# andrewcsmith/vox_box.rs

Hardware: AMD Instinct MI355X
Metric: frames/sec (pitch+LPC+formants), 48 kHz 25 ms/10 ms hop, 1→8 MI355X (higher is better)
Workload: dtype f64

## Files before the change

vox_box.rs_amd/csrc/vbx_pitch_refine.hpp:

```cpp
#pragma once
#include <type_traits>

#include "vbx_device.hpp"
#include "vbx_kernels.hpp"

namespace vbx {


__device__ __forceinline__ double fma_sc(double p, double x, const double c) {
    double r;
    asm("v_fma_f64 %0, %1, %2, %3" : "=v"(r) : "v"(p), "v"(x), "s"(c));
    return r;
}

__device__ __forceinline__ double sin_poly_q(double x) {
    const double x2 = x * x;
    double p = -1.9572941063391261231e-20;
    p = fma_sc(p, x2, 8.2206352466243297170e-18);
    p = fma_sc(p, x2, -2.8114572543455207632e-15);
    p = fma_sc(p, x2, 7.6471637318198164759e-13);
    p = fma_sc(p, x2, -1.6059043836821614599e-10);
    p = fma_sc(p, x2, 2.5052108385441718775e-08);
    p = fma_sc(p, x2, -2.7557319223985890653e-06);
    p = fma_sc(p, x2, 1.9841269841269841270e-04);
// ... 450 lines not shown
            if (rest & 3) sinc_stream_tail<NSTEP>(s, step, rest & 3);
        } else if (sel) run_set(s, c1);
        else run_set(s, c0);
        const double acc = s.acc0 + s.acc1;
        const double signed_acc = __hiloint2double(__double2hiint(acc) ^ sign_bit, __double2loint(acc));
        return group_sum<64>(signed_acc * k);
    };
    double v = readfirstlane_f64(a + golden * (b - a));
    double fv = eval(v);
    double x = v, w = v, fx = fv, fw = fv;
    const bool prunable = __any(a >= (double)(-offset));
    pruned = false;
    if (prunable && __any(((fv <= 1.) ? fv : 1.) < bar)) { pruned = true; terms += nterms_s; evals += nevals_s; return true; }
    for (int it = 1; it <= 60; it++) {
        const double range = b - a;
        const double middle_range = (a + b) * 0.5;
        const double tol_act = sqrt_epsilon * fabs(x) + tol / 3.;
        if (__any(fabs(x - middle_range) + range * 0.5 <= 2. * tol_act)) break;
        double new_step = __any(x < middle_range) ? golden * (b - x) : golden * (a - x);
        if (__any(fabs(x - w) >= tol_act)) {
            const double t = (x - w) * (fx - fv);
            double q = (x - v) * (fx - fw);
            double p = (x - v) * q - (x - w) * t;
            q = 2. * q - t;
            if (__any(q > 0.)) p = -p; else q = -q;
            if (__any((int)(fabs(p) < fabs(new_step * q)) & (int)(p > q * (a - x + 2. * tol_act)) & (int)(p < q * (b - x - 2. * tol_act)))) {
                asm volatile("" ::: "memory");
                new_step = p / q;
            }
        }
        if (__any(fabs(new_step) < tol_act)) new_step = __any(new_step > 0.) ? tol_act : -tol_act;
        const double t = readfirstlane_f64(x + new_step);
        const double ft = eval(t);
        nevals_s += 1u;
        if (__any(ft <= fx)) {
            if (__any(t < x)) { asm volatile(""); b = x; } else { asm volatile(""); a = x; }
            v = w; w = x; x = t;
            fv = fw; fw = fx; fx = ft;
        } else {
            if (__any(t < x)) { asm volatile(""); a = t; } else { asm volatile(""); b = t; }
            if (__any(ft <= fw || fabs(w - x) < eps)) {
                v = w; w = t;
                fv = fw; fw = ft;
            } else if (__any(ft <= fv || fabs(v - x) < eps || fabs(v - w) < eps)) {
                v = t;
                fv = ft;
            }
        }
        if (prunable && __any(fx < bar)) { pruned = true; break; }
    }
    terms += nterms_s; evals += nevals_s;
    if (!pruned) { xmid = x; ymid = fx; }
    return true;
}

constexpr int Y_PAD = 16;
#ifndef VBX_EXP_PB
#define VBX_EXP_PB 5
#endif
constexpr int PB = VBX_EXP_PB;
__device__ __forceinline__ double block_abs_sum(const double *yp) {
    double s = fabs(yp[0]) + fabs(yp[1]);
#pragma unroll
    for (int i = 2; i + 1 < PB; i += 2) s += fabs(yp[i]) + fabs(yp[i + 1]);
    if (PB & 1) s += fabs(yp[PB - 1]);
    return s;
}
typedef unsigned short cand_t;
constexpr int PG = 16;
constexpr int PNG = 64 / PG;
constexpr int GROUP_PATH_MIN_CAND = 32;
#ifndef VBX_EXP_RG
#define VBX_EXP_RG 16
#endif
#ifndef VBX_EXP_GROUP_KMAX
#define VBX_EXP_GROUP_KMAX 4
#endif
constexpr int RG = VBX_EXP_RG;
#ifndef VBX_EXP_DUAL_MIN_CAND
#define VBX_EXP_DUAL_MIN_CAND 6
#endif
constexpr int DUAL_MIN_CAND = VBX_EXP_DUAL_MIN_CAND;

__device__ __forceinline__ void cand_from_peak(const double *ys, int kk, double sample_rate, int offset,
                                               double &freq, double &nn, const bool f32 = false) {
    const double peak = ys[kk], peak_rev = ys[kk - 1], peak_fwd = ys[kk + 1];
    if (f32) {
#pragma clang fp contract(off)
        const double dr = 0.5 * (double)(float)(peak_fwd - peak_rev);
        const double d2r = 2. * peak - (double)(float)(peak_rev - peak_fwd);
        freq = (double)(float)(sample_rate / (double)(float)((double)kk + dr / d2r));
        nn = (double)(float)((double)(float)(sample_rate / freq) - (double)offset);
        return;
    }
    const double dr = 0.5 * (peak_fwd - peak_rev);
    const double d2r = 2. * peak - (peak_rev - peak_fwd);
    freq = sample_rate / ((double)kk + dr / d2r);
    nn = sample_rate / freq - (double)offset;
}

constexpr int BOUND_HEAD = 8;

__device__ __forceinline__ double taper_upper(double theta) {
    const double t = theta * theta;
    double p = fma(t, 2.48015873015873016e-05, -1.38888888888888894e-03);
    p = fma(p, t, 4.16666666666666644e-02);
    p = fma(p, t, -0.5);
    return fma(0.5, fma(p, t, 1.0), 0.5) * (1.0 + 1.0e-15);
}

__device__ __forceinline__ void abs_range_idx(int nblk, int i0, int i1, int &j0, int &j1) {
    i0 = (i0 < 0) ? 0 : i0;
    const int last = PB * nblk - 1;
    i1 = (i1 > last) ? last : i1;
    const bool empty = i1 < i0;
    j0 = empty ? 0 : (int)((unsigned)i0 / PB);
    j1 = empty ? 0 : (int)((unsigned)i1 / PB) + 1;
}
template <int STEP, int TB>
__device__ __forceinline__ double first_eval_tail(const double *p16, int nblk, int offset, int nl, int nr, int D, int lo0,
                                                  double phil, double phir, double hl, double hr) {
    double tail = 0.0;
    for (int lo = lo0; lo <= D;) {
        double sl[TB], sr[TB];
#pragma unroll
        for (int q = 0, l = lo; q < TB; q++, l *= STEP) {
            const int hi = (2 * l < D + 1) ? 2 * l : D + 1;
            int a0 = 0, a1 = 0, b0 = 0, b1 = 0;
            if (l <= D) {
                abs_range_idx(nblk, offset + nr - (hi - 1), offset + nr - l, a0, a1);
                abs_range_idx(nblk, offset + nl + l, offset + nl + hi - 1, b0, b1);
            }
            sl[q] = p16[a1] - p16[a0];
            sr[q] = p16[b1] - p16[b0];
        }
#pragma unroll
        for (int q = 0; q < TB; q++) {
            if (lo > D) break;
            const double pl = phil + (double)lo, pr = phir + (double)lo;
            const double cl = rcp_nr1(pl) * taper_upper(hl * pl);
            const double cr = rcp_nr1(pr) * taper_upper(hr * pr);
            tail = fma(cl, sl[q], tail);
            tail = fma(cr, sr[q], tail);
            lo *= STEP;
        }
    }
    return tail;
}

__device__ __forceinline__ double first_eval_bound(const double *ys, const double *p16, int nblk, int nvalid, int ylen,
                                                   int offset, int nx, double nn, int depth) {
    const double INF = __builtin_inf();
    if (nn == 0. || nn >= (double)nx || !(nn - 1. < nn + 1.)) return INF;
    double v0;
    {
#pragma clang fp contract(off)
        const double golden = 1. - 0.6180339887498948482045868343656381177203091798057628621;
        const double ba = nn - 1., bb = nn + 1.;
        if (!(ba >= (double)(-offset))) return INF;
        v0 = ba + golden * (bb - ba);
    }
    if (nx < 1 || v0 > (double)nx || v0 < 0.0) return INF;
    const double fl = floor(v0);
    const int nl = (int)fl, nr = nl + 1;
    const double phil = v0 - (double)nl, phir = 1.0 - phil;
    if (fabs(v0 - (double)nl) < 1.0e-10 || fabs(v0 - (double)nr) < 1.0e-10) return INF;
    int D = depth;
    if ((offset + nr) < D) D = ((offset + nr) < 0) ? 0 : (offset + nr);
    if ((offset + nl + D) >= nx) D = nx - offset + nl - 1;
    if (D < 0 || offset + nr >= ylen || D > offset + nr || offset + nl < 0 || offset + nl + D >= ylen) return INF;
    const double s0 = sin_poly(M_PI * fmin(phil, phir)) * 0.31830988618379067154;
    const double hl = M_PI * rcp_nr1(phil + (double)D), hr = M_PI * rcp_nr1(phir + (double)D);
    double head = 0.0;
    const int nh = (BOUND_HEAD < D + 1) ? BOUND_HEAD : D + 1;
    {
        double cl = cos_0_pi(hl * phil), cr = cos_0_pi(hr * phir);
        double dl = cos_0_pi(hl * (phil + 1.0)) - cl, dr = cos_0_pi(hr * (phir + 1.0)) - cr;
        const double sl = sin_poly(0.5 * hl), sr = sin_poly(0.5 * hr);
        const double kl = 4.0 * sl * sl, kr = 4.0 * sr * sr;
        double yl[BOUND_HEAD], yr[BOUND_HEAD];
#pragma unroll
// ... 15 lines not shown
        }
    }
    head *= s0;
    double tail = first_eval_tail<2, 4>(p16, nblk, offset, nl, nr, D, nh, phil, phir, hl, hr);
    tail *= s0;
    const double ub = head + tail * (1.0 + 1.0e-9) + (1.0e-9 + 1.0e-11 * p16[nblk]);
    return (ub != ub) ? INF : ub;
}

__device__ __forceinline__ double first_eval_bound_quad(const double *ys, const double *p16, int nblk, int nvalid, int ylen,
                                                        int offset, int nx, double nn, int depth, int sub, bool have) {
    const double INF = __builtin_inf();
    bool inf = !have;
    double v0 = 0.;
    if (!inf) {
        if (nn == 0. || nn >= (double)nx || !(nn - 1. < nn + 1.)) inf = true;
        else {
#pragma clang fp contract(off)
            const double golden = 1. - 0.6180339887498948482045868343656381177203091798057628621;
            const double ba = nn - 1., bb = nn + 1.;
            if (!(ba >= (double)(-offset))) inf = true;
            v0 = ba + golden * (bb - ba);
        }
    }
    if (!inf && (nx < 1 || v0 > (double)nx || v0 < 0.0)) inf = true;
    int nl = 0, nr = 1, D = 0;
    double phil = 0.5, phir = 0.5;
    if (!inf) {
        const double fl = floor(v0);
        nl = (int)fl; nr = nl + 1;
        phil = v0 - (double)nl; phir = 1.0 - phil;
        if (fabs(v0 - (double)nl) < 1.0e-10 || fabs(v0 - (double)nr) < 1.0e-10) inf = true;
        D = depth;
        if ((offset + nr) < D) D = ((offset + nr) < 0) ? 0 : (offset + nr);
        if ((offset + nl + D) >= nx) D = nx - offset + nl - 1;
        if (D < 0 || offset + nr >= ylen || D > offset + nr || offset + nl < 0 || offset + nl + D >= ylen) inf = true;
    }
    double head = 0.0, tail = 0.0;
    if (!inf) {
        const double s0 = sin_poly(M_PI * fmin(phil, phir)) * 0.31830988618379067154;
        const double hl = M_PI * rcp_nr1(phil + (double)D), hr = M_PI * rcp_nr1(phir + (double)D);
        const int nh = (BOUND_HEAD < D + 1) ? BOUND_HEAD : D + 1;
        double yl[BOUND_HEAD / 4], yr[BOUND_HEAD / 4];
#pragma unroll
        for (int j = 0; j < BOUND_HEAD / 4; j++) {
            const int m = sub + 4 * j;
            const bool in = m < nh;
            yl[j] = y_at_padded(ys, nvalid, in ? offset + nr - m : 0);
            yr[j] = y_at_padded(ys, nvalid, in ? offset + nl + m : 0);
        }
#pragma unroll
        for (int j = 0; j < BOUND_HEAD / 4; j++) {
            const int m = sub + 4 * j;
            if (m >= nh) break;
            const double pl = phil + (double)m, pr = phir + (double)m;
            const double tl = yl[j] * rcp_nr1(pl) * fma(0.5, cos_0_pi(hl * pl), 0.5);
            const double tr = yr[j] * rcp_nr1(pr) * fma(0.5, cos_0_pi(hr * pr), 0.5);
            const double t = tl + tr;
            head += (m & 1) ? -t : t;
        }
        head *= s0;
        tail = first_eval_tail<16, 2>(p16, nblk, offset, nl, nr, D, nh << sub, phil, phir, hl, hr);
        tail *= s0;
    }
    head = group_sum<4>(head);
    tail = group_sum<4>(tail);
    const double ub = head + tail * (1.0 + 1.0e-9) + (1.0e-9 + 1.0e-11 * p16[nblk]);
    return (inf || ub != ub) ? INF : ub;
}

__device__ __forceinline__ int pick_best(float *keys, int ncand, double bar, int lane) {
    double bv = -__builtin_inf(); int bi = 0x7fffffff;
    for (int i = lane; i < ncand; i += 64) { const double v = (double)keys[i]; if (v > bv) { bv = v; bi = i; } }
    const double gm = wave_max(bv);
    int pick = (bv == gm) ? bi : 0x7fffffff;
    for (int o = 32; o > 0; o >>= 1) { const int other = __shfl_xor(pick, o, 64); pick = (other < pick) ? other : pick; }
    if (pick == 0x7fffffff || !(gm >= bar)) return -1;
    if (lane == 0) keys[pick] = -__builtin_inff();
    wave_sync();
    return pick;
}


__device__ __forceinline__ int pick_best_pred(float *keys, const cand_t *cand_list, const double *ys, int ncand, double bar, int lane) {
    double bv = -__builtin_inf(); int bi = 0x7fffffff;
    for (int i = lane; i < ncand; i += 64) {
        const float kv = keys[i];
        if (kv > -__builtin_inff() && (double)kv >= bar) {
            const int k = (int)cand_list[i];
            double p = fmin(ys[k - 1], ys[k + 1]);
            if (!(p == p)) p = __builtin_inf();
            if (bi == 0x7fffffff || p > bv) { bv = p; bi = i; }
        }
    }
    const double gm = wave_max(bv);
    int pick = (bi != 0x7fffffff && bv == gm) ? bi : 0x7fffffff;
    for (int o = 32; o > 0; o >>= 1) { const int other = __shfl_xor(pick, o, 64); pick = (other < pick) ? other : pick; }
    if (pick == 0x7fffffff) return -1;
    if (lane == 0) keys[pick] = -__builtin_inff();
    wave_sync();
    return pick;
}


__host__ __device__ constexpr int pitch_refine_lds_bytes(int n, int nst = 0, int cap = 0) {
    const int m = (nst > 0) ? nst : n;
    return (m + Y_PAD + ((((m + PB - 1) / PB) + 2) & ~1)) * 8 + ((cap > 0) ? cap : n / 4 + 8) * (int)(sizeof(float) + sizeof(cand_t));
}

inline int pitch_curve_reach(int n, double sample_rate, double fmin) {
    if (!(fmin > 0.0) || !(sample_rate > 0.0)) return 0;
    const double reach = 2.0 * ceil(sample_rate / fmin) + 16.0;
    if (!(reach < (double)n)) return 0;
    return ((int)reach + 1) & ~1;
}
inline int pitch_curve_entries(int n, double sample_rate, double fmin) {
    if ((n & 1) || !(fmin > 0.0) || !(sample_rate > 0.0)) return 0;
    const double reach = 2.0 * ceil(sample_rate / fmin) + 16.0;
    if (!(reach < (double)n)) return 0;
    int m = (int)reach;
    if (m < n / 2 + 2) m = n / 2 + 2;
    m = (m + 1) & ~1;
    return (m < n) ? m : 0;
}

struct pitch_params_t { double sample_rate, threshold, fmin, fmax; int kmax; int full_off; int f32 = 0; int ncurve = 0; };
__host__ __device__ constexpr int pitch_full_list_entries(int n) { return n / 4 + 2; }

#ifndef VBX_EXP_CELL_NB_PITCH
#define VBX_EXP_CELL_NB_PITCH 0
#endif
#ifndef VBX_EXP_CELL_NB_REFINE_LIST
#define VBX_EXP_CELL_NB_REFINE_LIST 3
#endif
constexpr int PITCH_CELL_NB = VBX_EXP_CELL_NB_PITCH, REFINE_LIST_CELL_NB = VBX_EXP_CELL_NB_REFINE_LIST;
template <int STAGE = 0, int NB = 0>
__device__ __forceinline__ bool pitch_refine_store(double *ys, int n, const pitch_params_t &pp, long f,
                                                   double *__restrict__ out_cand, long cand_ld,
                                                   int32_t *__restrict__ out_count, int32_t *__restrict__ status,
                                                   unsigned long long *__restrict__ work, double unc_tol = 0.0,
                                                   double2 *full = nullptr, int *io_ncand = nullptr, int cand_cap = 0,
                                                   uint16_t *list_at = nullptr) {
    const int lane = lane_id();
    const double sample_rate = pp.sample_rate, threshold = pp.threshold, fmin = pp.fmin, fmax = pp.fmax;
    const int kmax = pp.kmax;
    const bool f32 = pp.f32 != 0;
    const int nst = (pp.ncurve > 0) ? pp.ncurve : n;
    const int nblk = (nst + PB - 1) / PB;
    double *p16 = ys + nst + Y_PAD;
    float *keys = reinterpret_cast<float *>(p16 + ((nblk + 2) & ~1));
    cand_t *cand_list = (STAGE == 1 && list_at != nullptr) ? reinterpret_cast<cand_t *>(list_at)
                                                           : reinterpret_cast<cand_t *>(keys + ((STAGE == 2 && cand_cap > 0) ? cand_cap : n / 4 + 8));
    const int b = (int)floor(0.5 * (double)n);
    const int offset = -b - 1;
    const int nx = b - offset;
    const int ylen = 2 * n;
    const int nvalid = nst + Y_PAD;

    VBX_PHASE_INIT();
    int ncand = 0;
    if constexpr (STAGE == 2) ncand = *io_ncand;
    else {
    int npeak = 0;
    bool unsure = false;
    for (int base = 0; base < b; base += 64) {
        const int k = base + lane;
        bool peak = false;
        if (k >= 1 && k + 1 < b) {
            const double c = ys[k];
            const double d1 = c - ys[k - 1], d2 = c - ys[k + 1];
            peak = (ys[k - 1] < c) && (ys[k + 1] < c);
            unsure = unsure || (fabs((d1 < d2) ? d1 : d2) <= unc_tol);
        }
        const unsigned long long mask = __ballot(peak);
        if (peak) cand_list[npeak + __popcll(mask & ((1ull << lane) - 1ull))] = (cand_t)k;
        npeak += __popcll(mask);
    }
    wave_sync();
    if (unc_tol > 0.0 && __any(unsure)) return false;
    VBX_PHASE(work, f, 6);
    unsure = false;
    for (int base = 0; base < npeak; base += 64) {
        const int i = base + lane;
        bool pass = false;
        int k = 0;
        if (i < npeak) {
            k = cand_list[i];
            double freq, nn;
            cand_from_peak(ys, k, sample_rate, offset, freq, nn, f32);
            pass = (freq == 0.0) || (freq > fmin && freq < fmax);
            if (unc_tol > 0.0) {
                const double c = ys[k], d2r = 2. * c - (ys[k - 1] - ys[k + 1]), dr = 0.5 * (ys[k + 1] - ys[k - 1]);
                const double dlag = unc_tol * (1.0 + 4.0 * fabs(dr / d2r)) / fabs(d2r);
                const double tol_f = 2.0 * freq * dlag / fabs((double)k + dr / d2r);
                if (!(fabs(freq - fmin) > tol_f && fabs(freq - fmax) > tol_f)) unsure = true;
            }
        }
        wave_sync();
        const unsigned long long mask = __ballot(pass);
        if (pass) cand_list[ncand + __popcll(mask & ((1ull << lane) - 1ull))] = (cand_t)k;
        ncand += __popcll(mask);
        wave_sync();
    }

    if (unc_tol > 0.0 && __any(unsure)) return false;
    VBX_PHASE(work, f, 7);
    }
    if constexpr (STAGE == 1) { *io_ncand = ncand; return true; }

    const bool in_order = full != nullptr || kmax > ncand || f32;
    if (!in_order) {
        const int per = (nblk + 63) >> 6;
        double tot = 0.0;
        for (int q = 0; q < per; q++) {
            const int j = lane * per + q;
            if (j < nblk) tot += block_abs_sum(ys + PB * j);
        }
        const double incl = wave_inclusive_scan(tot);
        double run = incl - tot;
        if (lane == 0) p16[0] = 0.0;
        for (int q = 0; q < per; q++) {
            const int j = lane * per + q;
            if (j < nblk) {
                run += block_abs_sum(ys + PB * j);
                p16[j + 1] = run;
            }
        }
        wave_sync();
        const bool quad = ((ncand + 15) / 16) * 7 < ((ncand + 63) / 64) * 25;
        if (quad) {
            for (int base = 0; base < ncand; base += 16) {
                const int c = base + (lane >> 2);
                const bool have = c < ncand;
                double freq = 0., nn = 0.;
                if (have) cand_from_peak(ys, cand_list[c], sample_rate, offset, freq, nn, f32);
                const double ub = first_eval_bound_quad(ys, p16, nblk, nvalid, ylen, offset, nx, nn, 1200, lane & 3, have);
                const double kb = (ub <= 1.) ? ub : ((ub != ub) ? __builtin_inf() : ((ub == __builtin_inf()) ? ub : 1.));
                if (have && (lane & 3) == 0) keys[c] = __double2float_ru(kb);
            }
        } else {
            for (int c = lane; c < ncand; c += 64) {
                double freq, nn;
                cand_from_peak(ys, cand_list[c], sample_rate, offset, freq, nn, f32);
                const double ub = first_eval_bound(ys, p16, nblk, nvalid, ylen, offset, nx, nn, 1200);
                const double kb = (ub <= 1.) ? ub : ((ub != ub) ? __builtin_inf() : ((ub == __builtin_inf()) ? ub : 1.));
                keys[c] = __double2float_ru(kb);
            }
        }
        wave_sync();
    }

    VBX_PHASE(work, f, 8);
    int st = 0;
    int kept = 0;
    double lf = 0.0, ls = 0.0;
    bool any_nan = false;
    int li = 0;
    { lf = 0.0; ls = threshold; li = ncand; kept = 1; }
    const bool fullm = full != nullptr;
    if (fullm && lane == 0) full[ncand] = double2{0.0, threshold};

#define VBX_BAR() ((!fullm && !f32 && kept == kmax) ? readlane_f64(ls, kmax - 1) : -__builtin_inf())
    auto insert = [&](double f_g, double s_g, int c_g) {
        if (s_g != s_g) any_nan = true;
        if (fullm) { if (lane == 0) full[c_g] = double2{f_g, s_g}; return; }
        const int pos = __popcll(__ballot(lane < kept && (ls > s_g || (ls == s_g && li < c_g))));
        const double pf = from_prev_lane(lf), ps = from_prev_lane(ls);
        const int pi = __builtin_amdgcn_update_dpp(0, li, DPP_WAVE_SHR1, 0xf, 0xf, true);
        if (lane > pos) { lf = pf; ls = ps; li = pi; }
        if (lane == pos) { lf = f_g; ls = s_g; li = c_g; }
        kept = (kept + 1 < kmax) ? kept + 1 : kmax;
    };
    unsigned cterms = 0, cevals = 0;

    int next_full = ncand - 1;
    unsigned nterms = 0, nevals = 0;
    int group_lanes = RG;
    if (ncand <= GROUP_PATH_MIN_CAND && !(kmax >= VBX_EXP_GROUP_KMAX && ncand >= 4)) {
        auto enter = [&](int c, double xmid, double ymid) __attribute__((always_inline)) {
            double xm, ym;
            {
#pragma clang fp contract(off)
                xm = xmid + (double)offset;
                ym = ymid;
                if (ym > 1.) ym = 1. / ym;
                xm = sample_rate / (f32 ? (double)(float)xm : xm);
                if (f32) { xm = (double)(float)xm; ym = (double)(float)ym; }
            }
            insert(xm, ym, c);
        };
        int c_general = -1;
#ifndef VBX_EXP_NO_WAVE_BRENT
        for (;;) {
            const double bar = VBX_BAR();
            const int c = in_order ? next_full-- : pick_best_pred(keys, cand_list, ys, ncand, bar, lane);
            if (c < 0) break;
            double freq, nn, xmid, ymid;
            cand_from_peak(ys, cand_list[c], sample_rate, offset, freq, nn, f32);
            bool dropped = false;
            if (__builtin_expect(!improve_extremum_sinc_wave<NB>(ys, nvalid, ylen, offset, nx, nn, 1200, xmid, ymid, cterms, cevals, bar, dropped), 0)) {
                c_general = c;
                break;
            }
            if (dropped) continue;
            enter(c, xmid, ymid);
        }
        if (c_general >= 0)
#endif
        for (;;) {
            const double bar = VBX_BAR();
            int c = c_general;
            c_general = -1;
            if (c < 0) c = in_order ? next_full-- : pick_best_pred(keys, cand_list, ys, ncand, bar, lane);
            if (c < 0) break;
            double freq, nn, xmid, ymid;
            cand_from_peak(ys, cand_list[c], sample_rate, offset, freq, nn, f32);
            bool dropped = false;
            improve_extremum_sinc<64>(ys, nvalid, ylen, offset, nx, nn, 1200, true, xmid, ymid, st, &cterms, &cevals, bar, &dropped);
            if (dropped) continue;
            enter(c, xmid, ymid);
        }
    } else {
      auto run_groups = [&](auto pg_tag, auto dual_tag) {
        constexpr int PG = decltype(pg_tag)::value;
        constexpr bool DUAL = decltype(dual_tag)::value;
        bool exhausted = false;
        const int gid = lane / PG;
        int ci = -1, it = 0;
        bool special = false, safe = false, trusted = false;
        double ba = 0., bb = 0., v = 0., w = 0., x = 0., fv = 0., fw = 0., fx = 0., xmid = 0., ymid = 0.;
        constexpr unsigned long long LEADERS = (PG == 16) ? 0x0001000100010001ull : (PG == 8) ? 0x0101010101010101ull
                                             : (PG == 32) ? 0x0000000100000001ull : (PG == 4) ? 0x1111111111111111ull : 1ull;
        const double golden = 1. - 0.6180339887498948482045868343656381177203091798057628621;
        const double sqrt_epsilon = 1.4901161193847656e-08, eps = 2.220446049250313e-16, tol = 1e-10;
        for (;;) {
#pragma clang fp contract(off)
            bool finished = false;
            double range = 0., middle_range = 0., tol_act = 0.;
            if (ci >= 0) {
                if (special) finished = true;
                else if (it > 0) {
                    range = bb - ba;
                    middle_range = (ba + bb) * 0.5;
                    tol_act = sqrt_epsilon * fabs(x) + tol / 3.;
                    if (it > 60 || fabs(x - middle_range) + range * 0.5 <= 2. * tol_act) { finished = true; xmid = x; ymid = fx; }
                }
            }
            if (__any(finished)) {
                unsigned long long fm = __ballot(finished) & LEADERS;
                double xm = xmid + (double)offset;
                double ym = ymid;
                if (ym > 1.) ym = 1. / ym;
                double cf = sample_rate / (f32 ? (double)(float)xm : xm), cs = ym;
                if (f32) { cf = (double)(float)cf; cs = (double)(float)cs; }
                while (fm) {
                    const int ld = __builtin_ctzll(fm);
                    fm &= fm - 1;
                    insert(readlane_f64(cf, ld), readlane_f64(cs, ld), __builtin_amdgcn_readlane(ci, ld));
                }
                if (finished) ci = -1;
            }
            {
                unsigned long long im = __ballot(ci < 0) & LEADERS;
                while (im != 0ull && !exhausted) {
                    const int c = in_order ? next_full-- : pick_best_pred(keys, cand_list, ys, ncand, VBX_BAR(), lane);
                    if (c < 0) { exhausted = true; break; }
                    const int g = __builtin_ctzll(im) / PG;
                    im &= im - 1ull;
                    if (gid == g) {
                        ci = c;
                        double freq, nn;
                        cand_from_peak(ys, cand_list[ci], sample_rate, offset, freq, nn, f32);
                        it = 0; special = false; xmid = 0.; ymid = 0.;
                        if (nn == 0.) { special = true; xmid = 0.; ymid = ys[0]; }
                        else if (nn >= (double)nx) { special = true; xmid = (double)nx; ymid = y_at(ys, nvalid, nx - 1); }
                        else if (!(nn - 1. < nn + 1.)) { special = true; st |= 4; }
                        ba = nn - 1.; bb = nn + 1.;
                        safe = ba >= (double)(-offset);
                        trusted = !special && sinc_bracket_trusted(ba, bb, nvalid, ylen, offset, nx, 1200);
                    }
                }
            }
            if (!__any(ci >= 0)) break;
            const double bar = VBX_BAR();

            bool need = false;
            double t = 0.;
            if (ci >= 0 && !special) {
                if (it == 0) { v = ba + golden * (bb - ba); t = v; }
                else {
                    double new_step = (x < middle_range) ? golden * (bb - x) : golden * (ba - x);
                    if (fabs(x - w) >= tol_act) {
                        const double tt = (x - w) * (fx - fv);
                        double q = (x - v) * (fx - fw);
                        double pp = (x - v) * q - (x - w) * tt;
                        q = 2. * q - tt;
                        if (q > 0.) pp = -pp; else q = -q;
                        if (fabs(pp) < fabs(new_step * q) && pp > q * (ba - x + 2. * tol_act) && pp < q * (bb - x - 2. * tol_act))
                            new_step = pp / q;
                    }
                    if (fabs(new_step) < tol_act) new_step = (new_step > 0.) ? tol_act : -tol_act;
                    t = x + new_step;
                }
                need = true;
            }
            const double ft = sinc_interp<PG, DUAL>(ys, nvalid, ylen, offset, nx, t, 1200, need, st, &nterms, trusted);
            nevals += need ? 1u : 0u;
            if (need) {
                if (it == 0) {
                    x = v; w = v; fv = ft; fx = ft; fw = ft; it = 1;
                    const double ub = (ft <= 1.) ? ft : 1.;
                    if (ub < bar && safe) ci = -1;
                } else {
                    if (ft <= fx) {
                        if (t < x) bb = x; else ba = x;
                        v = w; w = x; x = t;
                        fv = fw; fw = fx; fx = ft;
                    } else {
                        if (t < x) ba = t; else bb = t;
                        if (ft <= fw || fabs(w - x) < eps) {
                            v = w; w = t;
                            fv = fw; fw = ft;
                        } else if (ft <= fv || fabs(v - x) < eps || fabs(v - w) < eps) {
                            v = t;
                            fv = ft;
                        }
                    }
                    it++;
                    if (safe && fx < bar) ci = -1;
                }
            }
        }
      };
      const bool dual_ok = in_order || (kmax >= 8 && ncand >= 12);
      if (RG == 16 && dual_ok && ncand >= DUAL_MIN_CAND) { run_groups(std::integral_constant<int, RG / 2>{}, std::true_type{}); group_lanes = RG / 2; }
      else run_groups(std::integral_constant<int, RG>{}, std::false_type{});
    }
#undef VBX_BAR
    VBX_PHASE(work, f, 9);
    const int total_cand = ncand + 1;
    st = __any(st & 4) ? 4 : 0;
    if (total_cand > 1 && (any_nan || threshold != threshold)) st |= 8;
    int code = 0;
    if (st & 4) code = 4; else if (st & 8) code = 3;
    if (fullm) {
        wave_sync();
        if (pp.full_off < 0) {
            __builtin_amdgcn_fence(__ATOMIC_RELEASE, "agent");
            __builtin_amdgcn_fence(__ATOMIC_ACQUIRE, "agent");
// ... 44 lines not shown
```

vox_box.rs_amd/csrc/vbx_spectral_1200.hpp:

```cpp
#pragma once

#include <type_traits>
#include "vbx_device.hpp"
#include "vbx_kernels.hpp"
#include "vbx_mfcc_tail.hpp"
#include "vbx_mfcc_interp.hpp"
#include "vbx_pitch_refine.hpp"
#include "vbx_spectral.hpp"

namespace vbx {

constexpr int SP_N = SPECTRAL_N;
constexpr int SP_M = 2 * SP_N;
constexpr int SP_S1 = 61;
constexpr int SP_S2 = 404;
constexpr int SP_T1 = 0;
constexpr int SP_T2 = SP_T1 + 60 * 20;
constexpr int SP_TM = SP_T2 + 3 * 20;
static_assert(SP_TM + 601 == SPECTRAL_TAB_COMPLEX, "table layout");
constexpr int SP_T2_LDS_OFFSET = (2 * 602 + 64) * 8;
static_assert(SP_T2_LDS_OFFSET >= (20 * SP_S1 > 3 * SP_S2 ? 20 * SP_S1 : 3 * SP_S2) * 8 && SP_T2_LDS_OFFSET % 16 == 0, "T2 behind both");

__device__ __forceinline__ void dft5(double &r0, double &i0, double &r1, double &i1, double &r2, double &i2,
                                     double &r3, double &i3, double &r4, double &i4) {
// ... 73 lines not shown
        for (int k = 0; k < 10; k++) tw[k] = tab[SP_T1 + np * 20 + 10 * h + k];
#pragma unroll
        for (int k = 0; k < 10; k++) {
            if (10 * h + k == 0) continue;
            const int s = dft20_slot(10 * h + k);
            const double a = re[s], b = im[s];
            re[s] = fma(a, tw[k].x, -(b * tw[k].y));
            im[s] = fma(a, tw[k].y, b * tw[k].x);
        }
    }
    }
    const int ka2 = np % 20, c2 = np / 20;
    double br[20], bi[20];
    wave_sync();
#pragma unroll
    for (int k = 0; k < 20; k++) if (act) ex[k * SP_S1 + lane] = re[dft20_slot(k)];
    wave_sync();
#pragma unroll
    for (int b = 0; b < 20; b++) br[b] = ex[ka2 * SP_S1 + 3 * b + c2];
    wave_sync();
#pragma unroll
    for (int k = 0; k < 20; k++) if (act) ex[k * SP_S1 + lane] = im[dft20_slot(k)];
    wave_sync();
#pragma unroll
    for (int b = 0; b < 20; b++) bi[b] = ex[ka2 * SP_S1 + 3 * b + c2];
    dft20(br, bi);
    if constexpr (TIGHT) twiddle_tight<4>(br, bi, t2 + c2 * 20);
    else {
#pragma unroll
    for (int h = 0; h < 2; h++) {
        double2 tw[10];
#pragma unroll
        for (int k = 0; k < 10; k++) tw[k] = t2[c2 * 20 + 10 * h + k];
#pragma unroll
        for (int k = 0; k < 10; k++) {
            if (10 * h + k == 0) continue;
            const int s = dft20_slot(10 * h + k);
            const double a = br[s], b = bi[s];
            br[s] = fma(a, tw[k].x, -(b * tw[k].y));
            bi[s] = fma(a, tw[k].y, b * tw[k].x);
        }
    }
    }
    double vr[7][3], vi[7][3];
    wave_sync();
#pragma unroll
    for (int k = 0; k < 20; k++) if (act) ex[c2 * SP_S2 + ka2 + 20 * k] = br[dft20_slot(k)];
    wave_sync();
#pragma unroll
    for (int t = 0; t < 7; t++)
#pragma unroll
        for (int c = 0; c < 3; c++) vr[t][c] = (t < 6 || lane < 16) ? ex[c * SP_S2 + lane + 64 * t] : 0.0;
    wave_sync();
#pragma unroll
    for (int k = 0; k < 20; k++) if (act) ex[c2 * SP_S2 + ka2 + 20 * k] = bi[dft20_slot(k)];
    wave_sync();
#pragma unroll
    for (int t = 0; t < 7; t++)
#pragma unroll
        for (int c = 0; c < 3; c++) vi[t][c] = (t < 6 || lane < 16) ? ex[c * SP_S2 + lane + 64 * t] : 0.0;
    wave_sync();
    constexpr double H3 = 0.86602540378443864676;
#pragma unroll
    for (int t = 0; t < 7; t++) {
        const double sr = vr[t][1] + vr[t][2], si = vi[t][1] + vi[t][2];
        const double dr = vr[t][1] - vr[t][2], di = vi[t][1] - vi[t][2];
        xr[t][0] = vr[t][0] + sr; xi[t][0] = vi[t][0] + si;
        const double mr = fma(-0.5, sr, vr[t][0]), mi = fma(-0.5, si, vi[t][0]);
        xr[t][1] = fma(H3, di, mr); xi[t][1] = fma(-H3, dr, mi);
        if (KC == 3) { xr[t][2] = fma(-H3, di, mr); xi[t][2] = fma(H3, dr, mi); }
        else { xr[t][2] = 0.0; xi[t][2] = 0.0; }
    }
}

#ifndef VBX_SPECTRAL_WAVES
#define VBX_SPECTRAL_WAVES 2
#endif
#ifndef VBX_EXP_CELL_NB
#define VBX_EXP_CELL_NB 3
#endif
#ifndef VBX_EXP_CELL_NB_F32IN
#define VBX_EXP_CELL_NB_F32IN VBX_EXP_CELL_NB
#endif
__host__ __device__ constexpr int sp_cell_blocks(int waves, bool f32) { return f32 ? VBX_EXP_CELL_NB_F32IN : VBX_EXP_CELL_NB; }
template <bool LPC, bool MFCC, bool FULL, int MODE = SP_ANALYZE, int WAVES = VBX_SPECTRAL_WAVES, typename TIN = double>
__global__ __launch_bounds__(64) __attribute__((amdgpu_waves_per_eu(sp_is_mfcc_only(MODE) ? 2 : WAVES, sp_is_mfcc_only(MODE) ? 4 : WAVES))) void analyze_kernel(const spectral_args_t a) {
    constexpr bool F32 = std::is_same<TIN, float>::value;
    static_assert(!F32 || (FULL && MODE == SP_ANALYZE), "float samples: the fused analysis of full frames");
    static_assert(MODE != SP_MFCC_ONLY || (MFCC && FULL && !LPC), "the MFCC-only form needs the full frame and has no lag sums");
    static_assert(MODE != SP_AC_ONLY || (!MFCC && !LPC), "the autocorrelation-only form");
    static_assert(!sp_is_interp(MODE) || (MFCC && !FULL), "interpolated bins: a padded frame's MFCC");
    static_assert(MODE != SP_MFCC_ONLY_INTERP || !LPC, "the MFCC-only forms have no lag sums");
    constexpr bool PITCH = !sp_is_mfcc_only(MODE);
    constexpr bool INTERP = sp_is_interp(MODE);
    extern __shared__ __attribute__((aligned(16))) double smem[];
    const long f = xcd_item(blockIdx.x, a.n_frames);
    if (f >= a.n_frames) return;
    const int lane = lane_id();
    const int np = (lane < 60) ? lane : 59;
    const int n = FULL ? SP_N : a.n;
    double *ex = smem;
    const double *xf = a.frames + f * a.stride;
    double2 *t2 = reinterpret_cast<double2 *>(reinterpret_cast<char *>(smem) + SP_T2_LDS_OFFSET);
    VBX_PHASE_INIT();

    double re[20], im[20];
    const int16_t *x16 = reinterpret_cast<const int16_t *>(a.frames) + f * a.stride;
    const float *x32 = reinterpret_cast<const float *>(a.frames) + f * a.stride;
    {
        const bool al = ((((uintptr_t)xf) | ((uintptr_t)a.window)) & 15) == 0;
        double2 xv[10], wv[10];
        float2 xs32[F32 ? 10 : 1];
#pragma unroll
        for (int q = 0; q < 10; q++) {
            const int i = 120 * q + 2 * np;
            if constexpr (F32) {
                float lo, hi;
                if ((((uintptr_t)x32) & 7) == 0) { const float2 w = *reinterpret_cast<const float2 *>(x32 + i); lo = w.x; hi = w.y; }
                else { lo = x32[i]; hi = x32[i + 1]; }
                xs32[q] = float2{lo, hi};
                wv[q] = (a.window != nullptr) ? (((uintptr_t)a.window & 15) == 0 ? *reinterpret_cast<const double2 *>(a.window + i)
                                                                                  : double2{a.window[i], a.window[i + 1]}) : double2{1.0, 1.0};
            } else if (FULL && (a.pcm & SP_FLAG_PCM)) {
                int lo, hi;
                if ((((uintptr_t)x16) & 3) == 0) { const int w = *reinterpret_cast<const int *>(x16 + i); lo = (short)(w & 0xffff); hi = w >> 16; }
                else { lo = x16[i]; hi = x16[i + 1]; }
                xv[q] = double2{pcm16_value(lo), pcm16_value(hi)};
                wv[q] = (a.window != nullptr) ? (((uintptr_t)a.window & 15) == 0 ? *reinterpret_cast<const double2 *>(a.window + i)
                                                                                  : double2{a.window[i], a.window[i + 1]}) : double2{1.0, 1.0};
            } else if (al && i + 1 < n) {
                xv[q] = *reinterpret_cast<const double2 *>(xf + i);
                wv[q] = (a.window != nullptr) ? *reinterpret_cast<const double2 *>(a.window + i) : double2{1.0, 1.0};
            } else {
                xv[q] = double2{0.0, 0.0}; wv[q] = double2{1.0, 1.0};
                if (i < n) { xv[q].x = xf[i]; if (a.window != nullptr) wv[q].x = a.window[i]; }
                if (i + 1 < n) { xv[q].y = xf[i + 1]; if (a.window != nullptr) wv[q].y = a.window[i + 1]; }
            }
        }
#pragma unroll
        for (int q = 0; q < 10; q++) {
            if constexpr (F32) xv[q] = double2{(double)xs32[q].x, (double)xs32[q].y};
            re[q] = (a.window != nullptr) ? xv[q].x * wv[q].x : xv[q].x;
            im[q] = (a.window != nullptr) ? xv[q].y * wv[q].y : xv[q].y;
        }
#pragma unroll
        for (int q = 10; q < 20; q++) { re[q] = 0.0; im[q] = 0.0; }
    }
    const double x0 = readlane_f64(re[0], 0);
    if (lane < 60) t2[lane] = a.tab[SP_T2 + lane];
    VBX_PHASE(a.work, f, 0);

    double xr[7][3], xi[7][3];
    fft1200<3, (WAVES >= 3)>(re, im, xr, xi, ex, a.tab, t2);
    VBX_PHASE(a.work, f, 1);

    double ar[10], ai[10], br[10], bi[10];
#pragma unroll
    for (int t = 0; t < 7; t++)
#pragma unroll
        for (int kc = 0; kc < 3; kc++) if (t < 6 || lane < 16) ex[lane + 64 * t + 400 * kc] = xr[t][kc];
    wave_sync();
#pragma unroll
    for (int t = 0; t < 10; t++) {
        const int m = lane + 64 * t;
        const bool ok = m <= 600;
        ar[t] = ok ? ex[m] : 0.0;
// ... 219 lines not shown
    }
    if (LPC) {
        static_assert(SP_LPC_P == 12, "seven lanes hold r[0..12]");
        double *row = a.out_lpc + f * a.lpc_ld;
        if (lane < 7) { row[2 * lane] = r_e[0]; if (lane < 6) row[2 * lane + 1] = r_o[0]; }
    }
    double amax = -1.0;
#pragma unroll
    for (int s = 0; s < 11; s++) {
        const int i = 2 * jj[s];
        const double ae = fabs(r_e[s]), ao = fabs(r_o[s]);
        if (jj[s] >= 0 && i < n) amax = (ae > amax) ? ae : amax;
        if (jj[s] >= 0 && i + 1 < n) amax = (ao > amax) ? ao : amax;
    }
    amax = wave_max(amax);
    const double scale = 1.0 / amax;
    double *ys = smem;
    wave_sync();
    const bool by_table = (a.pcm & SP_FLAG_LAG_RCP) != 0 && fabs(scale) < 1e290 && fabs(scale) > 1e-290;
    const double *lag_rcp = a.lag_window + lag_rcp_offset(n);
    if (by_table) {
#ifndef VBX_EXP_LB
#define VBX_EXP_LB 4
#endif
        constexpr int LB = VBX_EXP_LB;
#pragma unroll
        for (int h = 0; h < (11 + LB - 1) / LB; h++) {
            double2 lwv[LB], rwv[LB];
#pragma unroll
            for (int u = 0; u < LB; u++) {
                const int s = LB * h + u;
                if (s >= 11) continue;
                const int i = 2 * jj[s];
                const int at = (jj[s] >= 0 && i + 1 < n) ? i : 0;
                lwv[u] = *reinterpret_cast<const double2 *>(a.lag_window + at);
                rwv[u] = *reinterpret_cast<const double2 *>(lag_rcp + at);
            }
#pragma unroll
            for (int u = 0; u < LB; u++) {
                const int s = LB * h + u;
                if (s >= 11) continue;
                const int i = 2 * jj[s];
                if (jj[s] >= 0 && i + 1 < n) {
                    double2 y;
                    y.x = quotient_by_table(r_e[s] * scale, lwv[u].x, rwv[u].x);
                    y.y = quotient_by_table(r_o[s] * scale, lwv[u].y, rwv[u].y);
                    *reinterpret_cast<double2 *>(ys + i) = y;
                } else if (jj[s] >= 0 && i < n) {
                    ys[i] = (r_e[s] * scale) / a.lag_window[i];
                }
            }
            asm volatile("" ::: "memory");
        }
    } else {
        double2 lwv[11];
#pragma unroll
        for (int s = 0; s < 11; s++) {
            const int i = 2 * jj[s];
            lwv[s] = *reinterpret_cast<const double2 *>(a.lag_window + ((jj[s] >= 0 && i + 1 < n) ? i : 0));
        }
#pragma unroll
        for (int s = 0; s < 11; s++) {
            const int i = 2 * jj[s];
            if (jj[s] >= 0 && i + 1 < n) {
                const double2 lw = lwv[s];
                double2 y;
                y.x = (r_e[s] * scale) / lw.x;
                y.y = (r_o[s] * scale) / lw.y;
                *reinterpret_cast<double2 *>(ys + i) = y;
            } else if (jj[s] >= 0 && i < n) {
                ys[i] = (r_e[s] * scale) / a.lag_window[i];
            }
        }
    }
    if (lane < Y_PAD) ys[n + lane] = 0.0;
#ifndef VBX_EXP_NO_EXACT_TAIL
    if (!FULL) spectral_exact_tail(ys, n, xf, a.window, a.lag_window, x0, scale, lane);
#endif
    wave_sync();
    VBX_PHASE(a.work, f, 5);
    const double unc_tol = SP_UNC_EPS * fabs(s0) * scale;
    double2 *full = a.pp.full_off > 0 ? reinterpret_cast<double2 *>(reinterpret_cast<char *>(smem) + a.pp.full_off)
                  : a.pp.full_off < 0 ? reinterpret_cast<double2 *>(a.out_cand + f * a.cand_ld) : nullptr;
    if (!pitch_refine_store<0, sp_cell_blocks(WAVES, F32)>(ys, n, a.pp, f, a.out_cand, a.cand_ld, a.out_count, a.pitch_status, a.work, unc_tol, full)) {
        if (lane == 0) a.unsure_list[atomicAdd(a.unsure_count, 1)] = (int32_t)f;
    }
}

}
```

Before: 39.79 million.

## Reuse candidate front-end results in pitch refine instead of recomputing

Adds a ONCE template path to pitch_refine_store that parks the first 16 candidates' nn values in LDS (the keys area) during candidate filtering, keeps them in registers after the quad bound pass, and reads them back with readlane instead of calling cand_from_peak again. It also holds the per-lane block absolute sums in registers so the prefix-sum pass does not recompute them, and gives pick_best_pred an early path that exits with a wave-wide any() when no candidate is eligible and ncand<=64. Debug stop macros (VBX_EXP_STOP) are added but are off by default. The cost is more register pressure and extra complexity, and the parked buffer reuses keys memory before the keys are written.

```diff
diff --git a/vox_box.rs_amd/csrc/vbx_pitch_refine.hpp b/vox_box.rs_amd/csrc/vbx_pitch_refine.hpp
--- a/vox_box.rs_amd/csrc/vbx_pitch_refine.hpp
+++ b/vox_box.rs_amd/csrc/vbx_pitch_refine.hpp
@@ -556,6 +556,9 @@
 #endif
 constexpr int DUAL_MIN_CAND = VBX_EXP_DUAL_MIN_CAND;
 
+__device__ __forceinline__ double nn_from_freq(double sample_rate, double freq, int offset) {
+    return sample_rate / freq - (double)offset;
+}
 __device__ __forceinline__ void cand_from_peak(const double *ys, int kk, double sample_rate, int offset,
                                                double &freq, double &nn, const bool f32 = false) {
     const double peak = ys[kk], peak_rev = ys[kk - 1], peak_fwd = ys[kk + 1];
@@ -570,7 +573,7 @@
     const double dr = 0.5 * (peak_fwd - peak_rev);
     const double d2r = 2. * peak - (peak_rev - peak_fwd);
     freq = sample_rate / ((double)kk + dr / d2r);
-    nn = sample_rate / freq - (double)offset;
+    nn = nn_from_freq(sample_rate, freq, offset);
 }
 
 constexpr int BOUND_HEAD = 8;
@@ -752,8 +755,20 @@
 }
 
 
+template <bool EARLY = false>
 __device__ __forceinline__ int pick_best_pred(float *keys, const cand_t *cand_list, const double *ys, int ncand, double bar, int lane) {
     double bv = -__builtin_inf(); int bi = 0x7fffffff;
+    if (EARLY && ncand <= 64) {
+        const float kv = (lane < ncand) ? keys[lane] : -__builtin_inff();
+        const bool eligible = kv > -__builtin_inff() && (double)kv >= bar;
+        if (!__any(eligible)) return -1;
+        if (eligible) {
+            const int k = (int)cand_list[lane];
+            double p = fmin(ys[k - 1], ys[k + 1]);
+            if (!(p == p)) p = __builtin_inf();
+            bv = p; bi = lane;
+        }
+    } else {
     for (int i = lane; i < ncand; i += 64) {
         const float kv = keys[i];
         if (kv > -__builtin_inff() && (double)kv >= bar) {
@@ -762,6 +777,7 @@
             if (!(p == p)) p = __builtin_inf();
             if (bi == 0x7fffffff || p > bv) { bv = p; bi = i; }
         }
+    }
     }
     const double gm = wave_max(bv);
     int pick = (bi != 0x7fffffff && bv == gm) ? bi : 0x7fffffff;
@@ -804,7 +820,12 @@
 #define VBX_EXP_CELL_NB_REFINE_LIST 3
 #endif
 constexpr int PITCH_CELL_NB = VBX_EXP_CELL_NB_PITCH, REFINE_LIST_CELL_NB = VBX_EXP_CELL_NB_REFINE_LIST;
-template <int STAGE = 0, int NB = 0>
+#ifndef VBX_EXP_STOP
+#define VBX_EXP_STOP 0
+#endif
+#define VBX_STOP_AT(k_) do { if (VBX_EXP_STOP == (k_)) return true; } while (0)
+#define VBX_STOP_AT_PICK(k_, c_) do { if (VBX_EXP_STOP == (k_)) { if (lane == 0 && out_count != nullptr) out_count[f] = (c_); return true; } } while (0)
+template <int STAGE = 0, int NB = 0, bool ONCE = false>
 __device__ __forceinline__ bool pitch_refine_store(double *ys, int n, const pitch_params_t &pp, long f,
                                                    double *__restrict__ out_cand, long cand_ld,
                                                    int32_t *__restrict__ out_count, int32_t *__restrict__ status,
@@ -827,6 +848,10 @@
     const int ylen = 2 * n;
     const int nvalid = nst + Y_PAD;
 
+    constexpr int NN_PARKED = 16;
+    constexpr bool NN_PARK = ONCE && STAGE == 0;
+    double *nn_park = reinterpret_cast<double *>(keys);
+    bool parked = false;
     VBX_PHASE_INIT();
     int ncand = 0;
     if constexpr (STAGE == 2) ncand = *io_ncand;
@@ -849,15 +874,19 @@
     wave_sync();
     if (unc_tol > 0.0 && __any(unsure)) return false;
     VBX_PHASE(work, f, 6);
+    VBX_STOP_AT(1);
     unsure = false;
+    parked = NN_PARK && !f32 && npeak <= 64 && n / 4 + 8 >= 2 * NN_PARKED;
     for (int base = 0; base < npeak; base += 64) {
         const int i = base + lane;
         bool pass = false;
         int k = 0;
+        double nn_i = 0.0;
         if (i < npeak) {
             k = cand_list[i];
             double freq, nn;
             cand_from_peak(ys, k, sample_rate, offset, freq, nn, f32);
+            if (parked) nn_i = nn_from_freq(sample_rate, freq, offset);
             pass = (freq == 0.0) || (freq > fmin && freq < fmax);
             if (unc_tol > 0.0) {
                 const double c = ys[k], d2r = 2. * c - (ys[k - 1] - ys[k + 1]), dr = 0.5 * (ys[k + 1] - ys[k - 1]);
@@ -868,19 +897,47 @@
         }
         wave_sync();
         const unsigned long long mask = __ballot(pass);
-        if (pass) cand_list[ncand + __popcll(mask & ((1ull << lane) - 1ull))] = (cand_t)k;
+        const int ci = ncand + __popcll(mask & ((1ull << lane) - 1ull));
+        if (pass) cand_list[ci] = (cand_t)k;
+        if (parked && pass && ci < NN_PARKED) nn_park[ci] = nn_i;
         ncand += __popcll(mask);
         wave_sync();
     }
 
     if (unc_tol > 0.0 && __any(unsure)) return false;
     VBX_PHASE(work, f, 7);
+    VBX_STOP_AT(2);
     }
     if constexpr (STAGE == 1) { *io_ncand = ncand; return true; }
 
     const bool in_order = full != nullptr || kmax > ncand || f32;
+    double nn_kept = 0.0;
+    int n_kept = 0;
     if (!in_order) {
         const int per = (nblk + 63) >> 6;
+        constexpr int PER_REG = 4;
+        if (ONCE && per <= PER_REG) {
+            double bs[PER_REG];
+            double tot = 0.0;
+#pragma unroll
+            for (int q = 0; q < PER_REG; q++) {
+                const int j = lane * per + q;
+                const bool in = q < per && j < nblk;
+                bs[q] = in ? block_abs_sum(ys + PB * j) : 0.0;
+                if (in) tot += bs[q];
+            }
+            const double incl = wave_inclusive_scan(tot);
+            double run = incl - tot;
+            if (lane == 0) p16[0] = 0.0;
+#pragma unroll
+            for (int q = 0; q < PER_REG; q++) {
+                const int j = lane * per + q;
+                if (q < per && j < nblk) {
+                    run += bs[q];
+                    p16[j + 1] = run;
+                }
+            }
+        } else {
         double tot = 0.0;
         for (int q = 0; q < per; q++) {
             const int j = lane * per + q;
@@ -896,14 +953,18 @@
                 p16[j + 1] = run;
             }
         }
+        }
         wave_sync();
+        VBX_STOP_AT(3);
         const bool quad = ((ncand + 15) / 16) * 7 < ((ncand + 63) / 64) * 25;
         if (quad) {
             for (int base = 0; base < ncand; base += 16) {
                 const int c = base + (lane >> 2);
                 const bool have = c < ncand;
                 double freq = 0., nn = 0.;
-                if (have) cand_from_peak(ys, cand_list[c], sample_rate, offset, freq, nn, f32);
+                if (parked && base == 0) { if (have) nn = nn_park[c]; }
+                else if (have) cand_from_peak(ys, cand_list[c], sample_rate, offset, freq, nn, f32);
+                if (ONCE && base == 0) { nn_kept = nn; n_kept = (ncand < 16) ? ncand : 16; }
                 const double ub = first_eval_bound_quad(ys, p16, nblk, nvalid, ylen, offset, nx, nn, 1200, lane & 3, have);
                 const double kb = (ub <= 1.) ? ub : ((ub != ub) ? __builtin_inf() : ((ub == __builtin_inf()) ? ub : 1.));
                 if (have && (lane & 3) == 0) keys[c] = __double2float_ru(kb);
@@ -921,6 +982,7 @@
     }
 
     VBX_PHASE(work, f, 8);
+    VBX_STOP_AT(4);
     int st = 0;
     int kept = 0;
     double lf = 0.0, ls = 0.0;
@@ -946,7 +1008,8 @@
     int next_full = ncand - 1;
     unsigned nterms = 0, nevals = 0;
     int group_lanes = RG;
-    if (ncand <= GROUP_PATH_MIN_CAND && !(kmax >= VBX_EXP_GROUP_KMAX && ncand >= 4)) {
+    if (VBX_EXP_STOP == 6) { }
+    else if (ncand <= GROUP_PATH_MIN_CAND && !(kmax >= VBX_EXP_GROUP_KMAX && ncand >= 4)) {
         auto enter = [&](int c, double xmid, double ymid) __attribute__((always_inline)) {
             double xm, ym;
             {
@@ -963,10 +1026,12 @@
 #ifndef VBX_EXP_NO_WAVE_BRENT
         for (;;) {
             const double bar = VBX_BAR();
-            const int c = in_order ? next_full-- : pick_best_pred(keys, cand_list, ys, ncand, bar, lane);
+            const int c = in_order ? next_full-- : pick_best_pred<ONCE>(keys, cand_list, ys, ncand, bar, lane);
+            VBX_STOP_AT_PICK(5, c);
             if (c < 0) break;
             double freq, nn, xmid, ymid;
-            cand_from_peak(ys, cand_list[c], sample_rate, offset, freq, nn, f32);
+            if (ONCE && c < n_kept) nn = readlane_f64(nn_kept, 4 * __builtin_amdgcn_readfirstlane(c));
+            else cand_from_peak(ys, cand_list[c], sample_rate, offset, freq, nn, f32);
             bool dropped = false;
             if (__builtin_expect(!improve_extremum_sinc_wave<NB>(ys, nvalid, ylen, offset, nx, nn, 1200, xmid, ymid, cterms, cevals, bar, dropped), 0)) {
                 c_general = c;
@@ -981,7 +1046,7 @@
             const double bar = VBX_BAR();
             int c = c_general;
             c_general = -1;
-            if (c < 0) c = in_order ? next_full-- : pick_best_pred(keys, cand_list, ys, ncand, bar, lane);
+            if (c < 0) c = in_order ? next_full-- : pick_best_pred<ONCE>(keys, cand_list, ys, ncand, bar, lane);
             if (c < 0) break;
             double freq, nn, xmid, ymid;
             cand_from_peak(ys, cand_list[c], sample_rate, offset, freq, nn, f32);
@@ -1033,8 +1098,8 @@
             {
                 unsigned long long im = __ballot(ci < 0) & LEADERS;
                 while (im != 0ull && !exhausted) {
-                    const int c = in_order ? next_full-- : pick_best_pred(keys, cand_list, ys, ncand, VBX_BAR(), lane);
-                    if (c < 0) { exhausted = true; break; }
+                    const int c = in_order ? next_full-- : pick_best_pred<ONCE>(keys, cand_list, ys, ncand, VBX_BAR(), lane);
+                    if (VBX_EXP_STOP == 5 || c < 0) { exhausted = true; break; }
                     const int g = __builtin_ctzll(im) / PG;
                     im &= im - 1ull;
                     if (gid == g) {
diff --git a/vox_box.rs_amd/csrc/vbx_spectral_1200.hpp b/vox_box.rs_amd/csrc/vbx_spectral_1200.hpp
--- a/vox_box.rs_amd/csrc/vbx_spectral_1200.hpp
+++ b/vox_box.rs_amd/csrc/vbx_spectral_1200.hpp
@@ -179,6 +179,12 @@
 #ifndef VBX_EXP_CELL_NB_F32IN
 #define VBX_EXP_CELL_NB_F32IN VBX_EXP_CELL_NB
 #endif
+#ifndef VBX_EXP_FRONT_END_ONCE
+#define VBX_EXP_FRONT_END_ONCE 1
+#endif
+__host__ __device__ constexpr bool sp_front_end_once(bool mfcc, bool full, int waves, bool f32) {
+    return VBX_EXP_FRONT_END_ONCE != 0 && !(!mfcc && full && waves >= 3 && !f32);
+}
 __host__ __device__ constexpr int sp_cell_blocks(int waves, bool f32) { return f32 ? VBX_EXP_CELL_NB_F32IN : VBX_EXP_CELL_NB; }
 template <bool LPC, bool MFCC, bool FULL, int MODE = SP_ANALYZE, int WAVES = VBX_SPECTRAL_WAVES, typename TIN = double>
 __global__ __launch_bounds__(64) __attribute__((amdgpu_waves_per_eu(sp_is_mfcc_only(MODE) ? 2 : WAVES, sp_is_mfcc_only(MODE) ? 4 : WAVES))) void analyze_kernel(const spectral_args_t a) {
@@ -564,7 +570,7 @@
     const double unc_tol = SP_UNC_EPS * fabs(s0) * scale;
     double2 *full = a.pp.full_off > 0 ? reinterpret_cast<double2 *>(reinterpret_cast<char *>(smem) + a.pp.full_off)
                   : a.pp.full_off < 0 ? reinterpret_cast<double2 *>(a.out_cand + f * a.cand_ld) : nullptr;
-    if (!pitch_refine_store<0, sp_cell_blocks(WAVES, F32)>(ys, n, a.pp, f, a.out_cand, a.cand_ld, a.out_count, a.pitch_status, a.work, unc_tol, full)) {
+    if (!pitch_refine_store<0, sp_cell_blocks(WAVES, F32), sp_front_end_once(MFCC, FULL, WAVES, F32)>(ys, n, a.pp, f, a.out_cand, a.cand_ld, a.out_count, a.pitch_status, a.work, unc_tol, full)) {
         if (lane == 0) a.unsure_list[atomicAdd(a.unsure_count, 1)] = (int32_t)f;
     }
 }
```

Result: faster. 40.35 million (median of 6 runs) (+1.4%).
